# yweweler/single-speaker-tts

Measured on AMD Instinct MI355X. Metric: mel-frames/sec (end-to-end text->waveform incl. 60-iter Griffin-Lim, 64-utt LJ-Speech-shaped batch per GPU), higher is better.
Workload: dtype f32

## Files before the change

single-speaker-tts_amd/csrc/api_handle.hip:

```cpp
#include "api_internal.h"

namespace tts_api {
thread_local std::string g_create_error;
const char* const kStageNames[ST_COUNT] = {"encoder", "decoder", "postnet", "denorm", "gl_iter", "gl_final", "debug_gemm", "eval_loss"};
}

namespace tts_api {


int fail(tts_handle_t h, int code, const std::string& msg) {
    if (h) h->err = msg;
    else g_create_error = msg;
    return code;
}


const char* kAtt = "decoder2/decoder/output_projection_wrapper/multi_rnn_cell/cell_0/attention_wrapper";

const char* kMrc = "decoder2/decoder/output_projection_wrapper/multi_rnn_cell";


std::string bn_name(int i) {
    return i == 0 ? std::string("batch_normalization") : "batch_normalization_" + std::to_string(i);
}
// ... 659 lines not shown
    h->gl_pending[0] = h->gl_pending[1] = false;
    h->gl_wide_used[0] = h->gl_wide_used[1] = false;
    {
        int rc = graph_drop(h);
        if (rc) return rc;
    }
    if (h->own_stream) hipStreamDestroy(h->stream);
    if (s) {
        h->stream = reinterpret_cast<hipStream_t>(s);
        h->own_stream = false;
    } else {
        HIPCHK(h, hipStreamCreate(&h->stream));
        h->own_stream = true;
    }
    return TTS_OK;
}


int tts_set_option(tts_handle_t h, const char* key, int value) {
    DeviceScope dev_scope(h);
    if (!h || !key) return TTS_ERR_INVALID;
    if (!std::strcmp(key, "use_graph")) {
        int have = 0;
        if (value && !(value == 2 && h->debug_hooks) && !graph_runtime_ok(&have))
            return fail(h, TTS_ERR_UNSUPPORTED,
                        "use_graph: this process runs the library on HIP runtime " + std::to_string(have) + ", older than the " +
                        std::to_string(HIP_VERSION) + " it was built with (a libamdhip64 loaded before the library, e.g. the one "
                        "PyTorch bundles); hipGraph replays of the decoder are wrong there (csrc/api_internal.h, `use_graph`) -- the "
                        "launches are enqueued directly instead");
        h->use_graph = value;
    }
    else if (!std::strcmp(key, "profile")) h->profile = value;
    else if (!std::strcmp(key, "fused_tail")) h->fused_tail = value;
    else if (!std::strcmp(key, "persistent_decoder")) {
        if (value != h->persistent_decoder) {
            int rc = sync_all(h);
            if (rc) return rc;
        }
        h->persistent_decoder = value;
    }
    else if (!std::strcmp(key, "gl_pair")) h->gl_pair = value;
    else if (!std::strcmp(key, "gl_wide_from")) h->gl_wide = value < -2 ? -2 : value;
    else if (!std::strcmp(key, "gemm_presplit") || !std::strcmp(key, "gemm_ps")) {
        if (value && !gemm_experiments_built())
            return fail(h, TTS_ERR_UNSUPPORTED, std::string(key) + ": a measured-and-not-faster GEMM variant of round 5; its kernels are only "
                        "in a tools build of gemm_f32.hip (-DGEMM_EXPERIMENTS, tools/build_variant.sh)");
        (key[5] == 'p' && key[6] == 'r' ? h->gemm_presplit : h->gemm_ps) = value;
    }
    else if (!std::strcmp(key, "pd_ws")) {
        if (value != h->pd_ws) {
            int rc = sync_all(h);
            if (rc) return rc;
        }
        h->pd_ws = value;
    }
    else if (!std::strcmp(key, "enc_stream")) {
        int rc = sync_all(h);
        if (rc) return rc;
        h->enc_stream = value;
    }
    else if (!std::strcmp(key, "debug_hooks")) h->debug_hooks = value;
    else if (!std::strcmp(key, "pd_debug_delay") || !std::strcmp(key, "gl_runs") || !std::strcmp(key, "gl_run_len") ||
             !std::strcmp(key, "timeline") || !std::strcmp(key, "gl_workers") || !std::strcmp(key, "pd_rows")) {
        if (!h->debug_hooks && value != 0)
            return fail(h, TTS_ERR_INVALID, std::string(key) + ": a test hook; set the option \"debug_hooks\" to 1 on this handle first");
        if (!std::strcmp(key, "pd_debug_delay")) h->pd_debug_delay = value;
// ... 334 lines not shown
```

single-speaker-tts_amd/csrc/api_internal.h:

```cpp
#pragma once
#include <cmath>
#include <cstdio>
#include <cstring>
#include <memory>
#include <mutex>
#include <string>
#include <utility>
#include <vector>
#include "decoder.h"
#include "griffin_lim.h"
#include "tts_common.h"
#include <algorithm>
#include <map>

namespace tts_api {
using namespace tts;


extern thread_local std::string g_create_error;

struct ManifestEntry {
    std::string name;
    std::vector<int64_t> shape;
    size_t numel() const {
// ... 13 lines not shown
    const float* lifter_wt;
    const float* lifter_b;
    std::vector<const float*> hw_wt, hw_b;
    const float* gru_in_wt;
    const float* gru_in_b;
    const float* gru_rec;
};

enum Stage { ST_ENCODER = 0, ST_DECODER, ST_POSTNET, ST_DENORM, ST_GL_ITER, ST_GL_FINAL, ST_DEBUG_GEMM, ST_EVAL_LOSS, ST_COUNT };
extern const char* const kStageNames[ST_COUNT];

struct ProfSpan {
    hipEvent_t a, b;
    int stage;
    int64_t launches;
};


}
using namespace tts_api;

#ifndef TTS_USE_GRAPH_DEFAULT
#define TTS_USE_GRAPH_DEFAULT 0
#endif
struct tts_handle_s {
    tts_config_t cfg;
    int device = 0;
    hipStream_t stream = nullptr;
    bool own_stream = false;
    std::string err;
    int use_graph = TTS_USE_GRAPH_DEFAULT;
    int fused_tail = 1;
    bool tail_configured = false;
    int profile = 0;
    int pipeline = 1;
    int reserve_cus = 32;
    int hold_lds_kb = 64;
    hipStream_t aux = nullptr;
    int* hold_flags = nullptr;
    hipEvent_t ev_aux = nullptr;
    unsigned call_count = 0;
    hipStream_t front = nullptr;
    hipStream_t encs = nullptr;
    int enc_stream = 1;
    hipEvent_t ev_enc_ready[2] = {nullptr, nullptr};
    hipEvent_t ev_dec_done[2] = {nullptr, nullptr};
    hipEvent_t ev_gap[2] = {nullptr, nullptr};
    bool enc_ready_pending[2] = {false, false}, dec_done_pending[2] = {false, false}, gap_pending[2] = {false, false};
    hipEvent_t ev_front_done = nullptr;
    hipEvent_t ev_post_done[2] = {nullptr, nullptr};
    bool post_pending[2] = {false, false};
    bool gl_wide_used[2] = {false, false};
    hipEvent_t ev_gl_done[2] = {nullptr, nullptr};
    bool gl_pending[2] = {false, false};
    bool front_pending = false;
    hipEvent_t ev_serial_done = nullptr;
    bool serial_pending = false;
    unsigned syn_calls = 0;
    int syn_shape[3] = {0, 0, 0};
    int last_enc_ahead = -1;
    bool in_synthesize = false;
    int persistent_decoder = 1;
    int pd_ws = 1;
    bool ws_configured = false;
    struct WeightImage { unsigned char* p = nullptr; size_t bytes = 0; int N = 0, K = 0, Cin = 0; };
    std::map<const float*, WeightImage> wimg;
// ... 178 lines not shown
        ProfSpan s{};
        if (hipEventCreate(&s.a) != hipSuccess || hipEventCreate(&s.b) != hipSuccess) return;
        s.stage = stage;
        s.launches = launches;
        hipEventRecord(s.a, h->stream);
        h->spans.push_back(s);
        idx = (int)h->spans.size() - 1;
    }
    ~ProfScope() {
        if (idx >= 0) hipEventRecord(h->spans[idx].b, h->stream);
    }
};

struct SynthScope {
    tts_handle_t h;
    explicit SynthScope(tts_handle_t h_) : h(h_) { h->in_synthesize = true; }
    ~SynthScope() { h->in_synthesize = false; }
};

int fail(tts_handle_t h, int code, const std::string& msg);
void build_manifest(tts_handle_t h);
int check_status(tts_handle_t h);
int sync_all(tts_handle_t h);
int graph_quiesce(tts_handle_t h);
int graph_drop(tts_handle_t h);
int ws_get(tts_handle_t h, const char* name, size_t bytes, void** out);
void prof_collect(tts_handle_t h);
GemmGroup dense_group(const float* A, int lda, const float* Wt, const float* bias, float* C, int ldc, int M, int N, int K, int act);
GemmGroup conv_group(const float* A, int Cin, int ktaps, int T, const float* Wt, const float* bias, const float* scale, const float* shift, float* C, int ldc, int coff, int M, int N, int act, int pool);
int gemm_attach_image(tts_handle_t h, GemmGroup& g, bool refresh = false);
void gemm_drop_images(tts_handle_t h);
int run_single(tts_handle_t h, const GemmGroup& g);
bool graph_runtime_ok(int* have);
int run_cbhg(tts_handle_t h, const CbhgWeights& w, const char* tag, const float* x, int B, int T, float* out, int64_t* launches);
int check_ready(tts_handle_t h);
int gl_tables(tts_handle_t h);
int device_cus(tts_handle_t h);
int stft_prepare(tts_handle_t h, int n, int win, int hop, int n_fft);
int stft_run(tts_handle_t h, const float* wav, int B, int n, int n_fft, int win, int hop, float2** out, int* Tf_out);
int gl_fp(int n_fft);
bool gl_is_streaming(int n_fft, int win, int hop);
int glg_twiddles(tts_handle_t h, int n_fft, const float2** out);
int glg_prepare(tts_handle_t h, int T, int win, int hop, int n_fft);
int gl_run_generic(tts_handle_t h, const float* mag_int, const float* init_ft, uint64_t seed, int B, int T, int n_iter, int win, int hop, int n_fft, float* wav, float* mse, bool peak_normalize);
int gl_prepare(tts_handle_t h, int T, int win, int hop, int n_fft);
int gl_run(tts_handle_t h, const float* mag_int, const float* init_ft, uint64_t seed, int B, int T, int n_iter, int win, int hop, int n_fft, float* wav, float* mse, bool peak_normalize = false, bool under_reservation = false, float2* const* phase_pair = nullptr, bool phase_ready = false, int wide_from = -1);
int standalone_begin(tts_handle_t h);
int standalone_end(tts_handle_t h);
int encoder_impl(tts_handle_t h, const int32_t* ids, int B, int Ts, float* memory);
int pd_kernel_for(tts_handle_t h, int B, int Ts, int budget);
int pd_choice(tts_handle_t h, int B, int Ts, int budget, bool pipelined);
int attention_keys(tts_handle_t h, const float* memory, int B, int Ts, float* keys);
int decoder_impl(tts_handle_t h, const float* memory, int B, int Ts, int n_steps, float* mel, float* alignments);
int postnet_impl(tts_handle_t h, const float* mel, int B, int T, float* linear, float* mag, float ref_db, float max_db, float power, int* db_flag = nullptr);
bool denorm_can_assert(float ref_db, float max_db);
int denorm_flag_arm(tts_handle_t h, int** flag);
int denorm_flag_read(tts_handle_t h);
int gl_wide_from(tts_handle_t h, int B, int Ts, int n_steps, int T, int n_iter);

#define WS(h, name, type, count, var)                                             \
    type* var = nullptr;                                                          \
    {                                                                             \
        void* _p = nullptr;                                                       \
        int _rc = ws_get(h, name, (size_t)(count) * sizeof(type), &_p);           \
        if (_rc != TTS_OK) return _rc;                                            \
        var = reinterpret_cast<type*>(_p);                                        \
    }
// ... 3 lines not shown
```

single-speaker-tts_amd/csrc/api_pipeline.hip:

```cpp
#include "api_internal.h"

namespace tts_api {


int gl_wide_from(tts_handle_t h, int B, int Ts, int n_steps, int T, int n_iter) {
    if (h->gl_wide == -2 || h->reserve_cus <= 0) return -1;
    const int pd = pd_choice(h, B, Ts, h->reserve_cus, true);
    if (pd == 0) return -1;
    if (h->gl_wide >= 0) return h->gl_wide;
    if (pd != 2) return -1;
    const int per_launch = h->gl_pair < 1 ? 1 : (h->gl_pair > 3 ? 3 : h->gl_pair);
    if (h->n_cus_dev != 256 || h->n_cus_dev - h->reserve_cus < 16) return -1;
    const double launch_ms = 3.125e-6 * (double)B * T * per_launch * 224.0 / (double)(h->n_cus_dev - h->reserve_cus);
    const double step_ms = (0.0356 + 0.0089 * (double)Ts / 150.0) * (h->cfg.force_cudnn ? 0.038 / 0.045 : 1.0);
    const double dec_ms = step_ms * n_steps + 0.1;
    const int n_launches = (n_iter + per_launch - 1) / per_launch;
    const int from = (int)std::ceil((dec_ms + 0.5 * launch_ms + 0.1) / launch_ms);
    return from <= n_launches ? from : -1;
}

}

extern "C" {

// ... 150 lines not shown
        HIPCHK(h, hipEventRecord(h->ev_dec_done[parity], h->front));
        h->dec_done_pending[parity] = true;
    }
    h->defer_projection = false;
    h->cur_hold_flag = nullptr;
    h->cur_cu_budget = 0;
    h->dec_chip_idle = false;
    h->stream = main_stream;
    if (!rc && !pipelined && h->front) {
        if (!h->ev_serial_done) HIPCHK(h, hipEventCreateWithFlags(&h->ev_serial_done, hipEventDisableTiming));
        HIPCHK(h, hipEventRecord(h->ev_serial_done, h->stream));
        h->serial_pending = true;
    }
    if (rc) {
        if (hold_flag) hipMemsetAsync(hold_flag, 1, sizeof(int), h->front);
        return rc;
    }
    const bool phase_on_front = gl_streaming && pipelined && sp->n_iter >= 0 && (init_phase != nullptr || sp->n_iter == 0);
    if (pipelined) {
        if (hold_flag) HIPCHK(h, hipMemsetAsync(hold_flag, 1, sizeof(int), h->front));
        if (phase_on_front) {
            if (h->gl_pending[parity]) HIPCHK(h, hipStreamWaitEvent(h->front, h->ev_gl_done[parity], 0));
            HIPCHK(h, launch_phase_init(h->front, init_phase, sp->seed, phase_pair[0], B, F, T, FP));
        }
        HIPCHK(h, hipEventRecord(h->ev_front_done, h->front));
        h->front_pending = true;
        HIPCHK(h, hipStreamWaitEvent(h->stream, h->ev_front_done, 0));
    }
    if (h->has_pending_proj) {
        h->has_pending_proj = false;
        if ((rc = run_single(h, h->pending_proj))) return rc;
    }
    if (h->encs) {
        HIPCHK(h, hipEventRecord(h->ev_gap[parity], h->stream));
        h->gap_pending[parity] = true;
    }
    int* db_flag = nullptr;
    if (denorm_can_assert(sp->ref_db, sp->max_db) && (rc = denorm_flag_arm(h, &db_flag))) return rc;
    if ((rc = postnet_impl(h, mel, B, T, linear, magi, sp->ref_db, sp->max_db, sp->power, db_flag))) return rc;
    if (db_flag && (rc = denorm_flag_read(h))) return rc;
    if (h->front) {
        HIPCHK(h, hipEventRecord(h->ev_post_done[parity], h->stream));
        h->post_pending[parity] = true;
    }
    const int wide_from = (pipelined && gl_streaming) ? gl_wide_from(h, B, Ts, sp->n_steps, T, sp->n_iter) : -1;
    h->gl_wide_used[parity] = wide_from >= 0;
    if (gl_streaming)
        rc = gl_run(h, magi, init_phase, sp->seed, B, T, sp->n_iter, sp->win_length, sp->hop_length, c.n_fft, wav, nullptr,
                    sp->peak_normalize != 0, pipelined, phase_pair, phase_on_front, wide_from);
    else
        rc = gl_run_generic(h, magi, init_phase, sp->seed, B, T, sp->n_iter, sp->win_length, sp->hop_length, c.n_fft, wav, nullptr,
                            sp->peak_normalize != 0);
    if (h->front && !rc) {
        HIPCHK(h, hipEventRecord(h->ev_gl_done[parity], h->stream));
        h->gl_pending[parity] = true;
    }
    return rc;
}



int tts_synthesize_host(tts_handle_t h, const int32_t* ids_host, int B, int Ts, const tts_synth_params_t* sp, int* ticket) {
    DeviceScope dev_scope(h);
    int rc = check_ready(h);
    if (rc) return rc;
    if (!ids_host || !sp || !ticket || B < 1 || Ts < 1 || sp->n_steps < 1)
        return fail(h, TTS_ERR_INVALID, "synthesize_host: bad arguments");
    auto& io = h->hio;
    const int T = sp->n_steps * h->cfg.reduction;
    const size_t ids_bytes = (size_t)B * Ts * sizeof(int32_t);
    const size_t n_wav = (size_t)B * sp->hop_length * (size_t)(T - 1);
    const bool want_lin = (sp->host_outputs & TTS_HOST_LINEAR) != 0, want_ali = (sp->host_outputs & TTS_HOST_ALIGNMENTS) != 0;
// ... 139 lines not shown
```

single-speaker-tts_amd/csrc/api_stages.hip:

```cpp
#include "api_internal.h"

namespace tts_api {


int run_cbhg(tts_handle_t h, const CbhgWeights& w, const char* tag, const float* x, int B, int T, float* out,
             int64_t* launches) {
    const tts_config_t& c = h->cfg;
    const int M = B * T;
    const int NB = w.n_banks, NF = w.n_filters;
    const int U = c.n_highway_units, H = c.n_gru_units;
    const std::string t(tag);
    WS(h, (t + ".bank").c_str(), float, (size_t)M * NB * NF, bank);
    WS(h, (t + ".p1").c_str(), float, (size_t)M * w.proj_filters[0], p1);
    WS(h, (t + ".p2").c_str(), float, (size_t)M * w.proj_filters[1], p2);
    WS(h, (t + ".hw0").c_str(), float, (size_t)M * U, hw0);
    WS(h, (t + ".hw1").c_str(), float, (size_t)M * U, hw1);
    WS(h, (t + ".xproj").c_str(), float, (size_t)M * 6 * H, xproj);

    for (int k0 = 0; k0 < NB; k0 += TTS_GEMM_MAX_GROUPS) {
        GemmBatch b;
        std::memset(&b, 0, sizeof(b));
        const int ng = std::min(TTS_GEMM_MAX_GROUPS, NB - k0);
        for (int i = 0; i < ng; ++i) {
            const int k = k0 + ng - 1 - i;
            b.g[i] = conv_group(x, w.c_in, k + 1, T, w.bank_wt[k], w.bank_b[k], w.bank_scale[k], w.bank_shift[k], bank,
                                NB * NF, k * NF, M, NF, ACT_RELU, 0);
        }
        for (int i = 0; i < ng; ++i) {
            int rc = gemm_attach_image(h, b.g[i]);
            if (rc) return rc;
        }
        b.ps = h->gemm_ps;
        HIPCHK(h, launch_gemm(h->stream, b, ng));
        ++*launches;
    }
    {
        GemmGroup g = conv_group(bank, NB * NF, 3, T, w.proj_wt[0], w.proj_b[0], w.proj_scale[0], w.proj_shift[0], p1,
                                 w.proj_filters[0], 0, M, w.proj_filters[0], ACT_RELU, 1);
        const int slices = gemm_splitk_slices(g.K);
        if (slices > 1) {
            WS(h, (t + ".splitk").c_str(), float, (size_t)slices * M * g.N, part);
            {
                int rc = gemm_attach_image(h, g);
                if (rc) return rc;
            }
            HIPCHK(h, launch_gemm_splitk(h->stream, g, slices, part, h->gemm_ps));
            ++*launches;
        } else {
            int rc = run_single(h, g);
            if (rc) return rc;
        }
        ++*launches;
    }
    {
        GemmGroup g = conv_group(p1, w.proj_filters[0], 3, T, w.proj_wt[1], w.proj_b[1], w.proj_scale[1],
                                 w.proj_shift[1], p2, w.proj_filters[1], 0, M, w.proj_filters[1], ACT_NONE, 0);
        g.R = x;
        g.ldr = w.c_in;
        int rc = run_single(h, g);
        if (rc) return rc;
        ++*launches;
    }
    if (h->fused_tail && cbhg_tail_supports(w.proj_filters[1], U, H, (int)w.hw_wt.size(), M)) {
        if (!h->tail_configured) {
            HIPCHK(h, cbhg_tail_configure());
            h->tail_configured = true;
        }
        CbhgTailParams tp;
        std::memset(&tp, 0, sizeof(tp));
        tp.X = p2; tp.ldx = w.proj_filters[1]; tp.c_in = w.proj_filters[1];
        tp.lifter_wt = w.lifter_wt; tp.lifter_b = w.lifter_b;
        tp.n_hw = (int)w.hw_wt.size();
        for (int l = 0; l < tp.n_hw; ++l) { tp.hw_wt[l] = w.hw_wt[l]; tp.hw_b[l] = w.hw_b[l]; }
        tp.gru_wt = w.gru_in_wt; tp.gru_b = w.gru_in_b;
        tp.hw_out = hw0; tp.xproj = xproj; tp.M = M;
        HIPCHK(h, launch_cbhg_tail(h->stream, tp));
        ++*launches;
    } else {
        {
            int rc = run_single(h, dense_group(p2, w.proj_filters[1], w.lifter_wt, w.lifter_b, hw0, U, M, U,
                                               w.proj_filters[1], ACT_RELU));
            if (rc) return rc;
            ++*launches;
        }
        float* cur = hw0;
        float* nxt = hw1;
        for (size_t l = 0; l < w.hw_wt.size(); ++l) {
            GemmGroup g = dense_group(cur, U, w.hw_wt[l], w.hw_b[l], nxt, U, M, 2 * U, U, ACT_NONE);
            g.epi = EPI_HIGHWAY;
            int rc = run_single(h, g);
            if (rc) return rc;
            ++*launches;
            std::swap(cur, nxt);
        }
        {
            int rc = run_single(h, dense_group(cur, U, w.gru_in_wt, w.gru_in_b, xproj, 6 * H, M, 6 * H, U, ACT_NONE));
            if (rc) return rc;
            ++*launches;
        }
    }
    HIPCHK(h, launch_bigru(h->stream, xproj, 6 * H, w.gru_rec, out, B, T, H, c.force_cudnn));
    ++*launches;
    return TTS_OK;
}


int check_ready(tts_handle_t h) {
    if (!h) return TTS_ERR_INVALID;
    if (!h->finalized) return fail(h, TTS_ERR_NOT_LOADED, "weights not loaded: call tts_finalize_weights first");
    return TTS_OK;
}


int gl_tables(tts_handle_t h) {
    auto& g = h->gl;
    if (g.configured) return TTS_OK;
    HIPCHK(h, gl_configure());
    std::vector<float2> t1(1024), t2(1024);
    for (int k = 0; k < 1024; ++k) {
        const double a1 = -2.0 * M_PI * k / 1024.0, a2 = -2.0 * M_PI * k / 2048.0;
        t1[k] = make_float2((float)std::cos(a1), (float)std::sin(a1));
        t2[k] = make_float2((float)std::cos(a2), (float)std::sin(a2));
    }
    HIPCHK(h, hipMalloc(&g.tw1024, 1024 * sizeof(float2)));
    HIPCHK(h, hipMalloc(&g.tw2048, 1024 * sizeof(float2)));
    HIPCHK(h, hipMemcpy(g.tw1024, t1.data(), 1024 * sizeof(float2), hipMemcpyHostToDevice));
    HIPCHK(h, hipMemcpy(g.tw2048, t2.data(), 1024 * sizeof(float2), hipMemcpyHostToDevice));
    {
        std::vector<float2> tb(1024 + 15 * 64);
        for (int k = 0; k < 1024; ++k) tb[k] = t2[k];
        for (int i = 0; i < 15 * 64; ++i) tb[1024 + i] = t1[(i & 63) * ((i >> 6) + 1)];
        HIPCHK(h, hipMalloc(&g.tables, tb.size() * sizeof(float2)));
        HIPCHK(h, hipMemcpy(g.tables, tb.data(), tb.size() * sizeof(float2), hipMemcpyHostToDevice));
    }
// ... 592 lines not shown
        if (defer_proj) {
            h->pending_proj = proj;
            h->has_pending_proj = true;
        } else if ((rc = run_single(h, proj))) {
            return rc;
        }
    }
    if (predictive) {
        int flag = 0;
        HIPCHK(h, hipMemcpyAsync(&flag, sc.err_flag, sizeof(int), hipMemcpyDeviceToHost, h->stream));
        HIPCHK(h, hipStreamSynchronize(h->stream));
        if (flag)
            return fail(h, TTS_ERR_UNSUPPORTED,
                        "LocalLuongAttention (predictive): a predicted attention window leaves the memory; the "
                        "reference pads such windows inconsistently and fails there too");
    }
    return TTS_OK;
}


int postnet_impl(tts_handle_t h, const float* mel, int B, int T, float* linear, float* mag, float ref_db,
                        float max_db, float power, int* db_flag) {
    int rc = check_ready(h);
    if (rc) return rc;
    if (!mel || (!linear && !mag) || B < 1 || T < 1) return fail(h, TTS_ERR_INVALID, "postnet_forward: bad arguments");
    const tts_config_t& c = h->cfg;
    const int M = B * T, H2 = 2 * c.n_gru_units, F = 1 + c.n_fft / 2;
    int64_t launches = 0;
    ProfScope ps(h, ST_POSTNET, 0);
    const float* dense_in = mel;
    int dense_k = c.n_mels;
    if (c.apply_post_processing) {
        WS(h, "post.gru", float, (size_t)M * H2, gru);
        if ((rc = run_cbhg(h, h->post, "post", mel, B, T, gru, &launches))) return rc;
        dense_in = gru;
        dense_k = H2;
    }
    GemmGroup g = dense_group(dense_in, dense_k, h->dense_wt, h->dense_b, linear, F, M, F, dense_k, ACT_NONE);
    if (mag) {
        g.C2 = mag;
        g.ldc2 = gl_fp(c.n_fft);
        g.N2 = gl_fp(c.n_fft);
        g.d_ref = ref_db;
        g.d_range = std::fabs(ref_db) + std::fabs(max_db);
        g.d_pow = power;
        g.d_flag = db_flag;
    }
    if ((rc = run_single(h, g))) return rc;
    ++launches;
    if (ps.idx >= 0) h->spans[ps.idx].launches = launches;
    return TTS_OK;
}


bool denorm_can_assert(float ref_db, float max_db) {
    return ref_db - (std::fabs(ref_db) + std::fabs(max_db)) < -100.0f;
}

int denorm_flag_arm(tts_handle_t h, int** flag) {
    if (!h->an.flag) HIPCHK(h, hipMalloc(&h->an.flag, sizeof(int)));
    HIPCHK(h, hipMemsetAsync(h->an.flag, 0, sizeof(int), h->stream));
    *flag = h->an.flag;
    return TTS_OK;
}

int denorm_flag_read(tts_handle_t h) {
    int flag = 0;
// ... 287 lines not shown
```

single-speaker-tts_amd/csrc/cbhg_tail.hip:

```cpp
#include "tts_common.h"

namespace tts {

#define CT_BM 128
#define CT_U 128
#define CT_XLD (CT_U + 4)
#define CT_BK 32
#define CT_BLD (CT_BK + 4)
#define CT_BN 256
#define CT_THREADS 512

#define CT_AIMG (3 * CT_BM * 64)
#define CT_BIMG (3 * CT_BN * 64)
size_t cbhg_tail_lds_bytes() { return (size_t)CT_BM * CT_XLD * sizeof(float) + CT_AIMG + CT_BIMG; }
typedef __bf16 ct_bf16x8_t __attribute__((ext_vector_type(8)));
__device__ __forceinline__ void ct_split3(float x, unsigned& h, unsigned& m, unsigned& l) {
    h = __float_as_uint(x);
    const float r1 = x - __uint_as_float(h & 0xFFFF0000u);
    m = __float_as_uint(r1);
    const float r2 = r1 - __uint_as_float(m & 0xFFFF0000u);
    l = __float_as_uint(r2);
}
__device__ __forceinline__ unsigned ct_pack_hi(unsigned a, unsigned b) { return __builtin_amdgcn_perm(b, a, 0x07060302u); }
__device__ __forceinline__ void ct_store_split4(unsigned char* img, int rows, int row, int kq, float4 v) {
    unsigned h[4], m[4], l[4];
    ct_split3(v.x, h[0], m[0], l[0]);
    ct_split3(v.y, h[1], m[1], l[1]);
    ct_split3(v.z, h[2], m[2], l[2]);
    ct_split3(v.w, h[3], m[3], l[3]);
    const int off = (row * 4 + ((kq >> 1) ^ ((row >> 2) & 3))) * 16 + (kq & 1) * 8;
    *reinterpret_cast<uint2*>(img + off) = make_uint2(ct_pack_hi(h[0], h[1]), ct_pack_hi(h[2], h[3]));
    *reinterpret_cast<uint2*>(img + rows * 64 + off) = make_uint2(ct_pack_hi(m[0], m[1]), ct_pack_hi(m[2], m[3]));
    *reinterpret_cast<uint2*>(img + 2 * rows * 64 + off) = make_uint2(ct_pack_hi(l[0], l[1]), ct_pack_hi(l[2], l[3]));
}

bool cbhg_tail_supports(int c_in, int units, int gru_units, int n_hw, long long M) {
    return units == CT_U && gru_units == 128 && c_in >= 4 && c_in <= CT_U && c_in % 4 == 0 && n_hw >= 0 && n_hw <= CBHG_TAIL_MAX_HW &&
           M >= 1 && (M + CT_BM) * 3 * CT_BN * (long long)sizeof(float) < 0xFFFFFFF0ll;
}

__global__ __launch_bounds__(CT_THREADS) void cbhg_tail_kernel(CbhgTailParams p) {
    extern __shared__ __attribute__((aligned(16))) float lds[];
    float* Xs = lds;
    unsigned char* Ai = reinterpret_cast<unsigned char*>(lds + CT_BM * CT_XLD);
    unsigned char* Bi = Ai + CT_AIMG;
    const int tid = threadIdx.x, lane = tid & 63, wave = tid >> 6;
    const int wm = wave & 1, wn = wave >> 1;
    const int li = lane & 31, lh = lane >> 5;
    const int m0 = blockIdx.x * CT_BM;
    const int M = p.M;

    {
        const __amdgpu_buffer_rsrc_t rs = __builtin_amdgcn_make_buffer_rsrc(const_cast<float*>(p.X), 0, (int)0xFFFFFFF0u, 0x00020000);
#pragma unroll
        for (int i = 0; i < (CT_BM * (CT_U / 4)) / CT_THREADS; ++i) {
            const int idx = tid + CT_THREADS * i;
            const int row = idx >> 5, c4 = idx & 31;
            const bool ok = m0 + row < M && 4 * c4 < p.c_in;
            const unsigned off = ok ? (unsigned)((size_t)(m0 + row) * p.ldx + 4 * c4) * 4u : 0xFFFFFFFFu;
            const float4 v = __builtin_bit_cast(float4, __builtin_amdgcn_raw_buffer_load_b128(rs, (int)off, 0, 0));
            *reinterpret_cast<float4*>(&Xs[row * CT_XLD + 4 * c4]) = v;
        }
    }

    const int n_jobs = 1 + p.n_hw + 3;
    const int kq = tid & 7;
    float4 rb[4];
    auto job_w = [&](int j) -> const float* {
        return j == 0 ? p.lifter_wt : (j <= p.n_hw ? p.hw_wt[j - 1] : p.gru_wt + (size_t)(j - 1 - p.n_hw) * CT_BN * CT_U);
    };
    auto job_k = [&](int j) { return j == 0 ? p.c_in : CT_U; };
    auto job_n = [&](int j) { return j == 0 ? CT_U : CT_BN; };
    auto load_chunk = [&](int j, int kc) {
        const __amdgpu_buffer_rsrc_t rs = __builtin_amdgcn_make_buffer_rsrc(const_cast<float*>(job_w(j)), 0, (int)0xFFFFFFF0u, 0x00020000);
        const int K = job_k(j), N = job_n(j);
        const int kk = kc * CT_BK + 4 * kq;
#pragma unroll
        for (int i = 0; i < 4; ++i) {
            const int row = (tid >> 3) + 64 * i;
            const bool ok = row < N && kk < K;
            rb[i] = __builtin_bit_cast(float4, __builtin_amdgcn_raw_buffer_load_b128(rs, ok ? (int)((unsigned)(row * K + kk) * 4u) : -1, 0, 0));
        }
    };
    auto stage_chunk = [&](int kc) {
#pragma unroll
        for (int i = 0; i < 4; ++i) ct_store_split4(Bi, CT_BN, (tid >> 3) + 64 * i, kq, rb[i]);
#pragma unroll
        for (int i = 0; i < 2; ++i) {
            const int row = (tid >> 3) + 64 * i;
            ct_store_split4(Ai, CT_BM, row, kq, *reinterpret_cast<const float4*>(&Xs[row * CT_XLD + kc * CT_BK + 4 * kq]));
        }
    };

    const __amdgpu_buffer_rsrc_t xp_rs = __builtin_amdgcn_make_buffer_rsrc(
        p.xproj, 0, (int)(unsigned)((size_t)M * 3 * CT_BN * sizeof(float) < 0xFFFFFFF0ull ? (size_t)M * 3 * CT_BN * sizeof(float) : 0xFFFFFFF0ull), 0x00020000);
    const __amdgpu_buffer_rsrc_t hw_rs = __builtin_amdgcn_make_buffer_rsrc(
        p.hw_out, 0, p.hw_out ? (int)(unsigned)((size_t)M * CT_U * sizeof(float)) : 0, 0x00020000);
    const int row_l = wm * 64 + 4 * lh;

    f32x16 acc[2][2];
    load_chunk(0, 0);
    for (int j = 0; j < n_jobs; ++j) {
        const int nch = (job_k(j) + CT_BK - 1) / CT_BK;
        const bool live = 64 * wn < job_n(j);
#pragma unroll
        for (int a = 0; a < 2; ++a)
#pragma unroll
            for (int b = 0; b < 2; ++b)
#pragma unroll
                for (int r = 0; r < 16; ++r) acc[a][b][r] = 0.f;
        for (int kc = 0; kc < nch; ++kc) {
            __syncthreads();
            stage_chunk(kc);
            __syncthreads();
            if (kc + 1 < nch) load_chunk(j, kc + 1);
            else if (j + 1 < n_jobs) load_chunk(j + 1, 0);
            if (live) {
#pragma unroll
                for (int q = 0; q < 2; ++q) {
                    const int ch = 2 * q + lh;
                    uint4 fa[2][3];
#pragma unroll
                    for (int tm = 0; tm < 2; ++tm) {
                        const int row = wm * 64 + tm * 32 + li;
                        const int off = (row * 4 + (ch ^ ((row >> 2) & 3))) * 16;
#pragma unroll
                        for (int sp = 0; sp < 3; ++sp) fa[tm][sp] = *reinterpret_cast<const uint4*>(Ai + sp * CT_BM * 64 + off);
                    }
#pragma unroll
                    for (int tn = 0; tn < 2; ++tn) {
                        const int row = wn * 64 + tn * 32 + li;
                        const int off = (row * 4 + (ch ^ ((row >> 2) & 3))) * 16;
                        uint4 fb[3];
#pragma unroll
                        for (int sp = 0; sp < 3; ++sp) fb[sp] = *reinterpret_cast<const uint4*>(Bi + sp * CT_BN * 64 + off);
#pragma unroll
                        for (int tm = 0; tm < 2; ++tm) {
#define CT_MMA(SA, SB)                                                                                                   \
                            acc[tm][tn] = __builtin_amdgcn_mfma_f32_32x32x16_bf16(__builtin_bit_cast(ct_bf16x8_t, fa[tm][SA]), \
                                                                                  __builtin_bit_cast(ct_bf16x8_t, fb[SB]), acc[tm][tn], 0, 0, 0);
                            CT_MMA(0, 2) CT_MMA(2, 0) CT_MMA(1, 1) CT_MMA(0, 1) CT_MMA(1, 0) CT_MMA(0, 0)
#undef CT_MMA
                        }
                    }
                }
            }
        }

        if (j == 0) {
            if (live) {
#pragma unroll
                for (int tn = 0; tn < 2; ++tn) {
                    const float b = p.lifter_b[wn * 64 + tn * 32 + li];
#pragma unroll
                    for (int tm = 0; tm < 2; ++tm)
#pragma unroll
                        for (int r = 0; r < 16; ++r) acc[tm][tn][r] = fmaxf(acc[tm][tn][r] + b, 0.f);
                }
            }
            __syncthreads();
            if (live) {
#pragma unroll
                for (int tn = 0; tn < 2; ++tn)
#pragma unroll
                    for (int tm = 0; tm < 2; ++tm)
#pragma unroll
                        for (int r = 0; r < 16; ++r) {
                            const int ro = tm * 32 + (r & 3) + 8 * (r >> 2);
                            Xs[(row_l + ro) * CT_XLD + wn * 64 + tn * 32 + li] = acc[tm][tn][r];
                        }
            }
        } else if (j <= p.n_hw) {
            const int unit = wn * 32 + li;
            const float bh = p.hw_b[j - 1][wn * 64 + li], bt = p.hw_b[j - 1][wn * 64 + 32 + li];
#pragma unroll
            for (int tm = 0; tm < 2; ++tm)
#pragma unroll
                for (int r = 0; r < 16; ++r) {
                    const int ro = tm * 32 + (r & 3) + 8 * (r >> 2);
                    const float hh = fmaxf(acc[tm][0][r] + bh, 0.f);
                    const float tt = sigmoidf_(acc[tm][1][r] + bt);
                    const float x = Xs[(row_l + ro) * CT_XLD + unit];
                    acc[tm][0][r] = hh * tt + x * (1.0f - tt);
                }
            __syncthreads();
#pragma unroll
            for (int tm = 0; tm < 2; ++tm)
#pragma unroll
                for (int r = 0; r < 16; ++r) {
                    const int ro = tm * 32 + (r & 3) + 8 * (r >> 2);
                    Xs[(row_l + ro) * CT_XLD + unit] = acc[tm][0][r];
                }
            if (j == p.n_hw) {
                const unsigned vb = (unsigned)((m0 + row_l) * CT_U + unit) * 4u;
#pragma unroll
                for (int tm = 0; tm < 2; ++tm)
#pragma unroll
                    for (int r = 0; r < 16; ++r) {
                        const int ro = tm * 32 + (r & 3) + 8 * (r >> 2);
                        const float y = acc[tm][0][r];
                        __builtin_amdgcn_raw_buffer_store_b32(__builtin_bit_cast(unsigned, y), hw_rs, (int)(vb + (unsigned)(ro * CT_U * 4)), 0, 0);
                    }
            }
        } else {
            const int pass = j - 1 - p.n_hw;
#pragma unroll
            for (int tn = 0; tn < 2; ++tn) {
                const int n = pass * CT_BN + wn * 64 + tn * 32 + li;
                const float b = p.gru_b[n];
                const unsigned vb = (unsigned)((m0 + row_l) * (3 * CT_BN) + n) * 4u;
#pragma unroll
                for (int tm = 0; tm < 2; ++tm)
#pragma unroll
                    for (int r = 0; r < 16; ++r) {
                        const int ro = tm * 32 + (r & 3) + 8 * (r >> 2);
                        const float y = acc[tm][tn][r] + b;
                        __builtin_amdgcn_raw_buffer_store_b32(__builtin_bit_cast(unsigned, y), xp_rs,
                                                              (int)(vb + (unsigned)(ro * 3 * CT_BN * 4)), 0, 0);
                    }
            }
        }
    }
    if (p.n_hw == 0 && p.hw_out) {
        __syncthreads();
        for (int idx = tid; idx < CT_BM * (CT_U / 4); idx += CT_THREADS) {
            const int row = idx >> 5, c4 = idx & 31;
            if (m0 + row < M)
                *reinterpret_cast<float4*>(&p.hw_out[(size_t)(m0 + row) * CT_U + 4 * c4]) = *reinterpret_cast<const float4*>(&Xs[row * CT_XLD + 4 * c4]);
        }
    }
}

hipError_t cbhg_tail_configure() {
    return hipFuncSetAttribute(reinterpret_cast<const void*>(&cbhg_tail_kernel), hipFuncAttributeMaxDynamicSharedMemorySize,
                               (int)cbhg_tail_lds_bytes());
}

hipError_t launch_cbhg_tail(hipStream_t s, const CbhgTailParams& p) {
// ... 7 lines not shown
```

single-speaker-tts_amd/csrc/gru.hip:

```cpp
#include "tts_common.h"

namespace tts {

#define GRU_THREADS 512
#define GRU_QPAD 36

template <int CTRL>
__device__ __forceinline__ float gru_dpp(float v) {
    return __builtin_bit_cast(float, __builtin_amdgcn_update_dpp(0, __builtin_bit_cast(int, v), CTRL, 0xF, 0xF, true));
}
__device__ __forceinline__ float gru_sum4(float v) {
    v += gru_dpp<0xB1>(v);
    v += gru_dpp<0x4E>(v);
    return v;
}
__device__ __forceinline__ void gru_lds_barrier() { asm volatile("s_waitcnt lgkmcnt(0)\n\ts_barrier" ::: "memory"); }
typedef float gru_f2 __attribute__((ext_vector_type(2)));
__device__ __forceinline__ gru_f2 gru_pk_fma(gru_f2 a, gru_f2 b, gru_f2 c) {
    gru_f2 d;
    asm("v_pk_fma_f32 %0, %1, %2, %3" : "=v"(d) : "v"(a), "v"(b), "v"(c));
    return d;
}
__device__ __forceinline__ float gru_dot32(const float* q, const gru_f2 (&w)[16]) {
    gru_f2 a = {0.f, 0.f}, b = {0.f, 0.f};
// ... 62 lines not shown
        float c;                                                                               \
        if (CUDNN) {  \
            c = tanhf_(X[2] + r * (gru_sum4(gru_dot32(hq, wc)) + bch));                        \
        } else {                                                                               \
            if (kq == 0) rhs[slot] = r * hreg;                                                 \
            gru_lds_barrier();                                                                 \
            c = tanhf_(X[2] + gru_sum4(gru_dot32(rhs + kq * GRU_QPAD, wc)));                   \
        }                                                                                      \
        hreg = u * hreg + (1.0f - u) * c;                                                      \
        if (kq == 0) {                                                                         \
            ob[(size_t)t * 2 * H] = hreg;                                                      \
            hs[(s + 1) & 1][slot] = hreg;                                                      \
        }                                                                                      \
        const float* xn = xrow(s + 3);                                                         \
        X[0] = xn[0]; X[1] = xn[H]; X[2] = xn[2 * H];                                          \
        ++s; t += dt;                                                                          \
        gru_lds_barrier();                                                                     \
    }
    while (s + 3 <= T) {
        GRU_STEP(xa)
        GRU_STEP(xb1)
        GRU_STEP(xc2)
    }
    if (s < T) GRU_STEP(xa)
    if (s < T) GRU_STEP(xb1)
#undef GRU_STEP
}

size_t bigru_wrec_floats(int H, int cudnn) {
    return 2 * ((size_t)H * 2 * H + (size_t)H * H + (cudnn ? H : 0));
}

hipError_t launch_bigru(hipStream_t s, const float* xproj, int xld, const float* wrec, float* out,
                        int B, int T, int H, int cudnn) {
    if (H != 128) return hipErrorInvalidValue;
    dim3 grid(B, 2);
    if (cudnn)
        hipLaunchKernelGGL((bigru_kernel<128, true>), grid, dim3(GRU_THREADS), 0, s, xproj, xld, wrec, out, B, T);
    else
        hipLaunchKernelGGL((bigru_kernel<128, false>), grid, dim3(GRU_THREADS), 0, s, xproj, xld, wrec, out, B, T);
    return hipGetLastError();
}

}
```

single-speaker-tts_amd/csrc/tts_common.h:

```cpp
#pragma once
#include <hip/hip_runtime.h>
#include <stdint.h>
#include <stddef.h>
#include <map>
#include <string>
#include <vector>

#include "../../include/sstts_hip.h"

namespace tts {

typedef float f32x4 __attribute__((ext_vector_type(4)));
typedef float f32x16 __attribute__((ext_vector_type(16)));

enum Act { ACT_NONE = 0, ACT_RELU = 1, ACT_SIGMOID = 2, ACT_TANH = 3 };
enum Epi { EPI_STD = 0, EPI_HIGHWAY = 1 };

__device__ __forceinline__ float sigmoidf_(float x) { return __builtin_amdgcn_rcpf(1.0f + __expf(-x)); }
__device__ __forceinline__ double wave_sum_f64(double v) {
#pragma unroll
    for (int o = 32; o > 0; o >>= 1) v += __shfl_xor(v, o);
    return v;
}
__device__ __forceinline__ void split_f64(double v, float* hi, float* lo) {
// ... 31 lines not shown
    const float* A;
    const int32_t* gather;
    int gather_rows;
    const float* Wt;
    const unsigned char* Wimg;
    const float* bias;
    const float* scale;
    const float* shift;
    const float* R;
    float* C;
    int M, N, K;
    int lda, T, Cin, padl, pool;
    int ldc, coff, ldr;
    int act, epi;
    float* C2;
    int ldc2, N2;
    float d_ref, d_range, d_pow;
    int* d_flag;
    int kt0, kt1;
};
#define TTS_GEMM_MAX_GROUPS 16
struct GemmBatch {
    GemmGroup g[TTS_GEMM_MAX_GROUPS];
    int ps;
};
hipError_t launch_gemm(hipStream_t s, const GemmBatch& b, int n_groups);
bool gemm_experiments_built();
hipError_t launch_gemm_splitk(hipStream_t s, const GemmGroup& g, int slices, float* partial, int ps = 0);
size_t gemm_weight_image_bytes(int N, int K);
hipError_t launch_gemm_pack_weights(hipStream_t s, const float* Wt, unsigned char* img, int N, int K, int Cin);
int gemm_splitk_slices(int K);

hipError_t launch_bigru(hipStream_t s, const float* xproj, int xld, const float* wrec, float* out,
                        int B, int T, int H, int cudnn);
size_t bigru_wrec_floats(int H, int cudnn);

#define CBHG_TAIL_MAX_HW 8
struct CbhgTailParams {
    const float* X; int ldx; int c_in;
    const float* lifter_wt; const float* lifter_b;
    const float* hw_wt[CBHG_TAIL_MAX_HW]; const float* hw_b[CBHG_TAIL_MAX_HW]; int n_hw;
    const float* gru_wt; const float* gru_b;
    float* hw_out;
    float* xproj;
    int M;
};
bool cbhg_tail_supports(int c_in, int units, int gru_units, int n_hw, long long M);
hipError_t cbhg_tail_configure();
hipError_t launch_cbhg_tail(hipStream_t s, const CbhgTailParams& p);

hipError_t cu_hold_configure();
hipError_t launch_cu_hold(hipStream_t s, int n_cus, const int* flag, double timeout_ms, int lds_kb = 64);

size_t eval_loss_partial_count(int B, int T, int n_mels, int F);
hipError_t launch_eval_loss(hipStream_t s, const float* mel_t, const float* mel_o, const float* lin_t, const float* lin_o, int B,
                            int T, int n_mels, int F, int max_blocks, double* partial, double* sums, float* losses);

struct DevBuf {
    void* p = nullptr;
    size_t bytes = 0;
};

}
```

Before: 4.439 million.

## Move postnet gap event to GRU launch, reserve LDS for bigru, optional proj2 fusion

The gap event that lets the encoder stream proceed is now recorded just before the postnet bidirectional GRU instead of before the whole postnet, so the next batch's front-end work can overlap the postnet convolutions. The postnet GRU launch requests 128 KB of dynamic LDS by default, which limits it to one block per CU so it gets exclusive CUs when the batch fits outside the reserved CUs. An optional path, off by default, fuses the second conv projection plus residual into the fused CBHG tail kernel and skips the p2 buffer. The trade-off is extra hipFuncSetAttribute calls and a possible change in co-scheduling and occupancy.

Result: no change. 4.479 million, median of 6 (+0.9%).

```diff
diff --git a/single-speaker-tts_amd/csrc/api_handle.hip b/single-speaker-tts_amd/csrc/api_handle.hip
--- a/single-speaker-tts_amd/csrc/api_handle.hip
+++ b/single-speaker-tts_amd/csrc/api_handle.hip
@@ -715,6 +715,12 @@
     }
     else if (!std::strcmp(key, "profile")) h->profile = value;
     else if (!std::strcmp(key, "fused_tail")) h->fused_tail = value;
+    else if (!std::strcmp(key, "tail_proj2")) h->tail_proj2 = value;
+    else if (!std::strcmp(key, "gap_at_gru")) h->gap_late = value;
+    else if (!std::strcmp(key, "gru_exclusive_kb")) {
+        if (value < 0 || value > 150) return fail(h, TTS_ERR_INVALID, "gru_exclusive_kb must be 0..150");
+        h->gru_exclusive_kb = value;
+    }
     else if (!std::strcmp(key, "persistent_decoder")) {
         if (value != h->persistent_decoder) {
             int rc = sync_all(h);
diff --git a/single-speaker-tts_amd/csrc/api_internal.h b/single-speaker-tts_amd/csrc/api_internal.h
--- a/single-speaker-tts_amd/csrc/api_internal.h
+++ b/single-speaker-tts_amd/csrc/api_internal.h
@@ -69,6 +69,10 @@
     int use_graph = TTS_USE_GRAPH_DEFAULT;
     int fused_tail = 1;
     bool tail_configured = false;
+    int tail_proj2 = 0;
+    int gap_late = 1;
+    int gru_exclusive_kb = 128;
+    hipEvent_t gap_at_gru = nullptr;
     int profile = 0;
     int pipeline = 1;
     int reserve_cus = 32;
@@ -313,7 +317,8 @@
 void gemm_drop_images(tts_handle_t h);
 int run_single(tts_handle_t h, const GemmGroup& g);
 bool graph_runtime_ok(int* have);
-int run_cbhg(tts_handle_t h, const CbhgWeights& w, const char* tag, const float* x, int B, int T, float* out, int64_t* launches);
+int run_cbhg(tts_handle_t h, const CbhgWeights& w, const char* tag, const float* x, int B, int T, float* out, int64_t* launches,
+             bool postnet = false);
 int check_ready(tts_handle_t h);
 int gl_tables(tts_handle_t h);
 int device_cus(tts_handle_t h);
diff --git a/single-speaker-tts_amd/csrc/api_pipeline.hip b/single-speaker-tts_amd/csrc/api_pipeline.hip
--- a/single-speaker-tts_amd/csrc/api_pipeline.hip
+++ b/single-speaker-tts_amd/csrc/api_pipeline.hip
@@ -206,12 +206,21 @@
         if ((rc = run_single(h, h->pending_proj))) return rc;
     }
     if (h->encs) {
+        if (h->gap_late && c.apply_post_processing) h->gap_at_gru = h->ev_gap[parity];
+        else HIPCHK(h, hipEventRecord(h->ev_gap[parity], h->stream));
+        h->gap_pending[parity] = true;
+    }
+    int* db_flag = nullptr;
+    if (denorm_can_assert(sp->ref_db, sp->max_db) && (rc = denorm_flag_arm(h, &db_flag))) {
+        h->gap_at_gru = nullptr;
+        return rc;
+    }
+    rc = postnet_impl(h, mel, B, T, linear, magi, sp->ref_db, sp->max_db, sp->power, db_flag);
+    if (h->gap_at_gru) {
+        h->gap_at_gru = nullptr;
         HIPCHK(h, hipEventRecord(h->ev_gap[parity], h->stream));
-        h->gap_pending[parity] = true;
-    }
-    int* db_flag = nullptr;
-    if (denorm_can_assert(sp->ref_db, sp->max_db) && (rc = denorm_flag_arm(h, &db_flag))) return rc;
-    if ((rc = postnet_impl(h, mel, B, T, linear, magi, sp->ref_db, sp->max_db, sp->power, db_flag))) return rc;
+    }
+    if (rc) return rc;
     if (db_flag && (rc = denorm_flag_read(h))) return rc;
     if (h->front) {
         HIPCHK(h, hipEventRecord(h->ev_post_done[parity], h->stream));
diff --git a/single-speaker-tts_amd/csrc/api_stages.hip b/single-speaker-tts_amd/csrc/api_stages.hip
--- a/single-speaker-tts_amd/csrc/api_stages.hip
+++ b/single-speaker-tts_amd/csrc/api_stages.hip
@@ -4,7 +4,8 @@
 
 
 int run_cbhg(tts_handle_t h, const CbhgWeights& w, const char* tag, const float* x, int B, int T, float* out,
-             int64_t* launches) {
+             int64_t* launches, bool postnet) {
+    bool fuse_p2 = postnet;
     const tts_config_t& c = h->cfg;
     const int M = B * T;
     const int NB = w.n_banks, NF = w.n_filters;
@@ -12,7 +13,14 @@
     const std::string t(tag);
     WS(h, (t + ".bank").c_str(), float, (size_t)M * NB * NF, bank);
     WS(h, (t + ".p1").c_str(), float, (size_t)M * w.proj_filters[0], p1);
-    WS(h, (t + ".p2").c_str(), float, (size_t)M * w.proj_filters[1], p2);
+    const bool tail = h->fused_tail && cbhg_tail_supports(w.proj_filters[1], U, H, (int)w.hw_wt.size(), M);
+    fuse_p2 = fuse_p2 && tail && h->tail_proj2 && w.proj_filters[1] == w.c_in &&
+              cbhg_tail_supports_p2(w.proj_filters[0], w.proj_filters[1], M);
+    float* p2 = nullptr;
+    if (!fuse_p2) {
+        WS(h, (t + ".p2").c_str(), float, (size_t)M * w.proj_filters[1], p2w);
+        p2 = p2w;
+    }
     WS(h, (t + ".hw0").c_str(), float, (size_t)M * U, hw0);
     WS(h, (t + ".hw1").c_str(), float, (size_t)M * U, hw1);
     WS(h, (t + ".xproj").c_str(), float, (size_t)M * 6 * H, xproj);
@@ -52,7 +60,7 @@
         }
         ++*launches;
     }
-    {
+    if (!fuse_p2) {
         GemmGroup g = conv_group(p1, w.proj_filters[0], 3, T, w.proj_wt[1], w.proj_b[1], w.proj_scale[1],
                                  w.proj_shift[1], p2, w.proj_filters[1], 0, M, w.proj_filters[1], ACT_NONE, 0);
         g.R = x;
@@ -61,7 +69,7 @@
         if (rc) return rc;
         ++*launches;
     }
-    if (h->fused_tail && cbhg_tail_supports(w.proj_filters[1], U, H, (int)w.hw_wt.size(), M)) {
+    if (tail) {
         if (!h->tail_configured) {
             HIPCHK(h, cbhg_tail_configure());
             h->tail_configured = true;
@@ -74,6 +82,12 @@
         for (int l = 0; l < tp.n_hw; ++l) { tp.hw_wt[l] = w.hw_wt[l]; tp.hw_b[l] = w.hw_b[l]; }
         tp.gru_wt = w.gru_in_wt; tp.gru_b = w.gru_in_b;
         tp.hw_out = hw0; tp.xproj = xproj; tp.M = M;
+        if (fuse_p2) {
+            tp.X = nullptr; tp.ldx = 0;
+            tp.P1 = p1; tp.c_p1 = w.proj_filters[0]; tp.T = T;
+            tp.p2_wt = w.proj_wt[1]; tp.p2_b = w.proj_b[1]; tp.p2_scale = w.proj_scale[1]; tp.p2_shift = w.proj_shift[1];
+            tp.R = x; tp.ldr = w.c_in; tp.n_p2 = w.proj_filters[1];
+        }
         HIPCHK(h, launch_cbhg_tail(h->stream, tp));
         ++*launches;
     } else {
@@ -99,7 +113,16 @@
             ++*launches;
         }
     }
-    HIPCHK(h, launch_bigru(h->stream, xproj, 6 * H, w.gru_rec, out, B, T, H, c.force_cudnn));
+    if (h->gap_at_gru && h->gap_late == 1) {
+        HIPCHK(h, hipEventRecord(h->gap_at_gru, h->stream));
+        h->gap_at_gru = nullptr;
+    }
+    const int excl = (postnet && 2 * B <= h->n_cus_dev - std::max(h->reserve_cus, 0)) ? h->gru_exclusive_kb * 1024 : 0;
+    HIPCHK(h, launch_bigru(h->stream, xproj, 6 * H, w.gru_rec, out, B, T, H, c.force_cudnn, excl));
+    if (h->gap_at_gru) {
+        HIPCHK(h, hipEventRecord(h->gap_at_gru, h->stream));
+        h->gap_at_gru = nullptr;
+    }
     ++*launches;
     return TTS_OK;
 }
@@ -758,7 +781,7 @@
     int dense_k = c.n_mels;
     if (c.apply_post_processing) {
         WS(h, "post.gru", float, (size_t)M * H2, gru);
-        if ((rc = run_cbhg(h, h->post, "post", mel, B, T, gru, &launches))) return rc;
+        if ((rc = run_cbhg(h, h->post, "post", mel, B, T, gru, &launches, true))) return rc;
         dense_in = gru;
         dense_k = H2;
     }
diff --git a/single-speaker-tts_amd/csrc/cbhg_tail.hip b/single-speaker-tts_amd/csrc/cbhg_tail.hip
--- a/single-speaker-tts_amd/csrc/cbhg_tail.hip
+++ b/single-speaker-tts_amd/csrc/cbhg_tail.hip
@@ -34,6 +34,11 @@
     *reinterpret_cast<uint2*>(img + 2 * rows * 64 + off) = make_uint2(ct_pack_hi(l[0], l[1]), ct_pack_hi(l[2], l[3]));
 }
 
+bool cbhg_tail_supports_p2(int c_p1, int n_p2, long long M) {
+    return c_p1 >= CT_BK && c_p1 % CT_BK == 0 && n_p2 >= 4 && n_p2 <= CT_U && n_p2 % 4 == 0 &&
+           (M + 1) * 3 * (long long)c_p1 * (long long)sizeof(float) < 0xFFFFFFF0ll && (long long)n_p2 * 3 * c_p1 * sizeof(float) < 0xFFFFFFF0ll;
+}
+
 bool cbhg_tail_supports(int c_in, int units, int gru_units, int n_hw, long long M) {
     return units == CT_U && gru_units == 128 && c_in >= 4 && c_in <= CT_U && c_in % 4 == 0 && n_hw >= 0 && n_hw <= CBHG_TAIL_MAX_HW &&
            M >= 1 && (M + CT_BM) * 3 * CT_BN * (long long)sizeof(float) < 0xFFFFFFF0ll;
@@ -50,7 +55,8 @@
     const int m0 = blockIdx.x * CT_BM;
     const int M = p.M;
 
-    {
+    const int jp = p.P1 ? 1 : 0;
+    if (!jp) {
         const __amdgpu_buffer_rsrc_t rs = __builtin_amdgcn_make_buffer_rsrc(const_cast<float*>(p.X), 0, (int)0xFFFFFFF0u, 0x00020000);
 #pragma unroll
         for (int i = 0; i < (CT_BM * (CT_U / 4)) / CT_THREADS; ++i) {
@@ -63,32 +69,56 @@
         }
     }
 
-    const int n_jobs = 1 + p.n_hw + 3;
+    const int n_jobs = jp + 1 + p.n_hw + 3;
     const int kq = tid & 7;
-    float4 rb[4];
+    float4 rb[4], ra[2];
     auto job_w = [&](int j) -> const float* {
+        if (j < jp) return p.p2_wt;
+        j -= jp;
         return j == 0 ? p.lifter_wt : (j <= p.n_hw ? p.hw_wt[j - 1] : p.gru_wt + (size_t)(j - 1 - p.n_hw) * CT_BN * CT_U);
     };
-    auto job_k = [&](int j) { return j == 0 ? p.c_in : CT_U; };
-    auto job_n = [&](int j) { return j == 0 ? CT_U : CT_BN; };
+    auto job_k = [&](int j) { return j < jp ? 3 * p.c_p1 : (j == jp ? p.c_in : CT_U); };
+    auto job_n = [&](int j) { return j < jp ? p.n_p2 : (j == jp ? CT_U : CT_BN); };
+    unsigned p2_taps[2] = {0u, 0u};
+    if (jp) {
+#pragma unroll
+        for (int i = 0; i < 2; ++i) {
+            const int m = m0 + (tid >> 3) + 64 * i;
+            const int t = m < M ? m % p.T : 0;
+            for (int tap = 0; tap < 3; ++tap)
+                if (m < M && t + tap - 1 >= 0 && t + tap - 1 < p.T) p2_taps[i] |= 1u << tap;
+        }
+    }
     auto load_chunk = [&](int j, int kc) {
         const __amdgpu_buffer_rsrc_t rs = __builtin_amdgcn_make_buffer_rsrc(const_cast<float*>(job_w(j)), 0, (int)0xFFFFFFF0u, 0x00020000);
         const int K = job_k(j), N = job_n(j);
-        const int kk = kc * CT_BK + 4 * kq;
+        const int tap = j < jp ? kc % 3 : 0;
+        const int ch = j < jp ? (kc / 3) * CT_BK + 4 * kq : 0;
+        const int kk = j < jp ? tap * p.c_p1 + ch : kc * CT_BK + 4 * kq;
 #pragma unroll
         for (int i = 0; i < 4; ++i) {
             const int row = (tid >> 3) + 64 * i;
             const bool ok = row < N && kk < K;
             rb[i] = __builtin_bit_cast(float4, __builtin_amdgcn_raw_buffer_load_b128(rs, ok ? (int)((unsigned)(row * K + kk) * 4u) : -1, 0, 0));
         }
+        if (j < jp) {
+            const __amdgpu_buffer_rsrc_t as = __builtin_amdgcn_make_buffer_rsrc(const_cast<float*>(p.P1), 0, (int)0xFFFFFFF0u, 0x00020000);
+#pragma unroll
+            for (int i = 0; i < 2; ++i) {
+                const int m = m0 + (tid >> 3) + 64 * i;
+                const bool ok = (p2_taps[i] >> tap) & 1u;
+                ra[i] = __builtin_bit_cast(float4, __builtin_amdgcn_raw_buffer_load_b128(
+                    as, ok ? (int)((unsigned)((m + tap - 1) * p.c_p1 + ch) * 4u) : -1, 0, 0));
+            }
+        }
     };
-    auto stage_chunk = [&](int kc) {
+    auto stage_chunk = [&](int j, int kc) {
 #pragma unroll
         for (int i = 0; i < 4; ++i) ct_store_split4(Bi, CT_BN, (tid >> 3) + 64 * i, kq, rb[i]);
 #pragma unroll
         for (int i = 0; i < 2; ++i) {
             const int row = (tid >> 3) + 64 * i;
-            ct_store_split4(Ai, CT_BM, row, kq, *reinterpret_cast<const float4*>(&Xs[row * CT_XLD + kc * CT_BK + 4 * kq]));
+            ct_store_split4(Ai, CT_BM, row, kq, j < jp ? ra[i] : *reinterpret_cast<const float4*>(&Xs[row * CT_XLD + kc * CT_BK + 4 * kq]));
         }
     };
 
@@ -111,7 +141,7 @@
                 for (int r = 0; r < 16; ++r) acc[a][b][r] = 0.f;
         for (int kc = 0; kc < nch; ++kc) {
             __syncthreads();
-            stage_chunk(kc);
+            stage_chunk(j, kc);
             __syncthreads();
             if (kc + 1 < nch) load_chunk(j, kc + 1);
             else if (j + 1 < n_jobs) load_chunk(j + 1, 0);
@@ -147,7 +177,35 @@
             }
         }
 
-        if (j == 0) {
+        if (j < jp) {
+            if (live) {
+                const __amdgpu_buffer_rsrc_t r_rs = __builtin_amdgcn_make_buffer_rsrc(
+                    const_cast<float*>(p.R), 0, (int)(unsigned)((size_t)M * p.ldr * sizeof(float)), 0x00020000);
+#pragma unroll
+                for (int tn = 0; tn < 2; ++tn) {
+                    const int n = wn * 64 + tn * 32 + li;
+                    const bool nok = n < p.n_p2;
+                    const float bv = nok ? p.p2_b[n] : 0.f;
+                    const float sc = nok ? p.p2_scale[n] : 0.f;
+                    const float sh = nok ? p.p2_shift[n] : 0.f;
+                    unsigned vb[4];
+#pragma unroll
+                    for (int q = 0; q < 4; ++q) vb[q] = (unsigned)((m0 + row_l + q) * p.ldr + (nok ? n : 0)) * 4u;
+#pragma unroll
+                    for (int tm = 0; tm < 2; ++tm)
+#pragma unroll
+                        for (int r = 0; r < 16; ++r) {
+                            const int ro = tm * 32 + (r & 3) + 8 * (r >> 2);
+                            const float res = __builtin_bit_cast(float, __builtin_amdgcn_raw_buffer_load_b32(
+                                r_rs, (int)vb[r & 3], (tm * 32 + 8 * (r >> 2)) * p.ldr * 4, 0));
+                            float v = acc[tm][tn][r] + bv;
+                            v = v * sc + sh;
+                            v += res;
+                            Xs[(row_l + ro) * CT_XLD + n] = (nok && m0 + row_l + ro < M) ? v : 0.f;
+                        }
+                }
+            }
+        } else if (j == jp) {
             if (live) {
 #pragma unroll
                 for (int tn = 0; tn < 2; ++tn) {
@@ -170,9 +228,9 @@
                             Xs[(row_l + ro) * CT_XLD + wn * 64 + tn * 32 + li] = acc[tm][tn][r];
                         }
             }
-        } else if (j <= p.n_hw) {
+        } else if (j - jp <= p.n_hw) {
             const int unit = wn * 32 + li;
-            const float bh = p.hw_b[j - 1][wn * 64 + li], bt = p.hw_b[j - 1][wn * 64 + 32 + li];
+            const float bh = p.hw_b[j - jp - 1][wn * 64 + li], bt = p.hw_b[j - jp - 1][wn * 64 + 32 + li];
 #pragma unroll
             for (int tm = 0; tm < 2; ++tm)
 #pragma unroll
@@ -191,7 +249,7 @@
                     const int ro = tm * 32 + (r & 3) + 8 * (r >> 2);
                     Xs[(row_l + ro) * CT_XLD + unit] = acc[tm][0][r];
                 }
-            if (j == p.n_hw) {
+            if (j - jp == p.n_hw) {
                 const unsigned vb = (unsigned)((m0 + row_l) * CT_U + unit) * 4u;
 #pragma unroll
                 for (int tm = 0; tm < 2; ++tm)
@@ -203,7 +261,7 @@
                     }
             }
         } else {
-            const int pass = j - 1 - p.n_hw;
+            const int pass = j - jp - 1 - p.n_hw;
 #pragma unroll
             for (int tn = 0; tn < 2; ++tn) {
                 const int n = pass * CT_BN + wn * 64 + tn * 32 + li;
diff --git a/single-speaker-tts_amd/csrc/gru.hip b/single-speaker-tts_amd/csrc/gru.hip
--- a/single-speaker-tts_amd/csrc/gru.hip
+++ b/single-speaker-tts_amd/csrc/gru.hip
@@ -118,13 +118,19 @@
 }
 
 hipError_t launch_bigru(hipStream_t s, const float* xproj, int xld, const float* wrec, float* out,
-                        int B, int T, int H, int cudnn) {
+                        int B, int T, int H, int cudnn, int lds_reserve) {
     if (H != 128) return hipErrorInvalidValue;
     dim3 grid(B, 2);
+    const void* k = cudnn ? reinterpret_cast<const void*>(&bigru_kernel<128, true>) : reinterpret_cast<const void*>(&bigru_kernel<128, false>);
+    if (lds_reserve > 0) {
+        hipError_t e = hipFuncSetAttribute(k, hipFuncAttributeMaxDynamicSharedMemorySize, lds_reserve);
+        if (e != hipSuccess) return e;
+    }
+    const size_t dyn = lds_reserve > 0 ? (size_t)lds_reserve : 0;
     if (cudnn)
-        hipLaunchKernelGGL((bigru_kernel<128, true>), grid, dim3(GRU_THREADS), 0, s, xproj, xld, wrec, out, B, T);
+        hipLaunchKernelGGL((bigru_kernel<128, true>), grid, dim3(GRU_THREADS), dyn, s, xproj, xld, wrec, out, B, T);
     else
-        hipLaunchKernelGGL((bigru_kernel<128, false>), grid, dim3(GRU_THREADS), 0, s, xproj, xld, wrec, out, B, T);
+        hipLaunchKernelGGL((bigru_kernel<128, false>), grid, dim3(GRU_THREADS), dyn, s, xproj, xld, wrec, out, B, T);
     return hipGetLastError();
 }
 
diff --git a/single-speaker-tts_amd/csrc/tts_common.h b/single-speaker-tts_amd/csrc/tts_common.h
--- a/single-speaker-tts_amd/csrc/tts_common.h
+++ b/single-speaker-tts_amd/csrc/tts_common.h
@@ -87,7 +87,7 @@
 int gemm_splitk_slices(int K);
 
 hipError_t launch_bigru(hipStream_t s, const float* xproj, int xld, const float* wrec, float* out,
-                        int B, int T, int H, int cudnn);
+                        int B, int T, int H, int cudnn, int lds_reserve = 0);
 size_t bigru_wrec_floats(int H, int cudnn);
 
 #define CBHG_TAIL_MAX_HW 8
@@ -99,8 +99,12 @@
     float* hw_out;
     float* xproj;
     int M;
+    const float* P1; int c_p1; int T;
+    const float* p2_wt; const float* p2_b; const float* p2_scale; const float* p2_shift;
+    const float* R; int ldr; int n_p2;
 };
 bool cbhg_tail_supports(int c_in, int units, int gru_units, int n_hw, long long M);
+bool cbhg_tail_supports_p2(int c_p1, int n_p2, long long M);
 hipError_t cbhg_tail_configure();
 hipError_t launch_cbhg_tail(hipStream_t s, const CbhgTailParams& p);
 
```
